# usexfg/xfg-stark

Hardware: AMD Instinct MI355X
Metric: burn-proofs/sec (2^16-step trace, blowup=8) (higher is better)
Workload: dtype u64; 1 GPU; batch of 64 burn proofs per GPU (configs[2]; configs[3] = 512 proofs on 8 GPUs); trace_length=65536, blowup=8, proof_options=42/8/4/None/8/31, parallelism=dp1 (independent proofs; RCCL scatter of inputs, gather of proof bytes), submission=pipelined, depth 6 (xfg_prove_batch_submit / xfg_batch_wait)

## Files before the change

### include/xfg_stark.h

```cpp
#ifndef XFG_STARK_H
#define XFG_STARK_H
#include <stddef.h>
#include <stdint.h>
#ifdef __cplusplus
extern "C" {
#endif

typedef struct xfg_ctx xfg_ctx;

typedef enum {
    XFG_OK = 0,
    XFG_INVALID_BURN_AMOUNT = 1,
    XFG_MINT_MISMATCH = 2,
    XFG_ZERO_TX_HASH = 3,
    XFG_BAD_RECIPIENT_LEN = 4,
    XFG_SHORT_SECRET = 5,
    XFG_PROVER_ERROR = 6,
    XFG_DEVICE_ERROR = 7,
    XFG_BUFFER_TOO_SMALL = 8,
    XFG_INVALID_ARGUMENT = 9,
    XFG_VERIFY_FAILED = 10,
    XFG_INVALID_TRACE = 11
} xfg_status;

// ... 135 lines not shown
                             const uint64_t* coeffs, const uint32_t* coin_seeds, const uint64_t* coin_counters,
                             uint64_t ginv, uint64_t* ood_out, uint64_t* deep_out, uint64_t* dp_out,
                             uint32_t* seeds_out, uint64_t* counters_out, int* fail_out);
int xfg_debug_constraint_eval(xfg_ctx* ctx, uint32_t count, uint64_t n, uint32_t blowup, uint32_t ext,
                              const uint64_t* trace, const xfg_air_consts* airs, const uint64_t* coeffs,
                              uint64_t* ce);
int xfg_debug_fri_fold(xfg_ctx* ctx, uint32_t count, uint32_t ext, uint32_t logn, uint32_t logbeta, int coset_major,
                       const uint64_t* vals, const uint64_t* alpha, uint64_t* out);
int xfg_debug_fri_fold_f(xfg_ctx* ctx, uint32_t count, uint32_t ext, uint32_t logn, uint32_t logbeta, int coset_major,
                         uint32_t fold, const uint64_t* vals, const uint64_t* alpha, uint64_t* out);
int xfg_debug_coin_draws(xfg_ctx* ctx, const uint32_t seed[8], uint64_t counter, uint32_t k, uint32_t ext,
                         const uint64_t reject[4], uint64_t* out_wave, uint64_t* out_seq, uint64_t counters[2],
                         int ok[2]);
int xfg_debug_merkle_lde(xfg_ctx* ctx, uint32_t count, uint32_t nc, uint64_t n, uint32_t blowup, const uint64_t* lde,
                         const uint64_t* entries, uint64_t nentries, uint8_t* nodes_out, uint8_t* local_out);
int xfg_debug_merkle_lde_const(xfg_ctx* ctx, uint32_t count, uint32_t nc, uint64_t n, uint32_t blowup,
                               const uint64_t* lde, const uint8_t* flags, const uint64_t* vals,
                               const uint64_t* entries, uint64_t nentries, uint8_t* nodes_out, uint8_t* local_out);
int xfg_debug_poison_lde(xfg_ctx* ctx, int on);
int xfg_debug_merkle_fri(xfg_ctx* ctx, uint32_t count, uint32_t ext, uint32_t logn, uint32_t logbeta, int coset_major,
                         const uint64_t* vals, uint8_t* nodes_out);
int xfg_debug_merkle_fri_f(xfg_ctx* ctx, uint32_t count, uint32_t ext, uint32_t logn, uint32_t logbeta, int coset_major,
                           uint32_t fold, const uint64_t* vals, uint8_t* nodes_out);
int xfg_debug_grind(xfg_ctx* ctx, uint32_t count, const uint32_t* seeds, uint32_t grind, uint64_t first_nonce,
                    uint64_t max_nonce, uint32_t chunk_log, uint32_t blocks, uint64_t* nonces_out);
int xfg_grind_probe(const xfg_ctx* ctx, uint32_t* device_min, uint64_t* device_searches, uint64_t* host_searches);
int xfg_debug_verify_batch_gpu(xfg_ctx* ctx, uint32_t count, const uint8_t* const* proofs, const size_t* lens,
                               const xfg_air_consts* airs, const xfg_options* acceptable, int* results,
                               uint64_t* flags, char* errs, size_t err_stride);

#ifdef __cplusplus
}
#endif
#endif
```

### xfg-stark_amd/csrc/debug_abi.hip

```cpp
#include <cstring>
#include <vector>

#include "dev_coin.hpp"
#include "dispatch.hpp"
#include "field_dft.hpp"
#include "prover_internal.hpp"

using namespace xfg;

__global__ void field_op_kernel(int op, const u64* a, const u64* b, u64* out, u64 count) {
    const u64 i = (u64)blockIdx.x * blockDim.x + threadIdx.x;
    if (i >= count) return;
    const u64 x = a[i], y = b[i];
    u64 r = 0;
    switch (op) {
        case 0: r = gl_mul(x, y); break;
        case 1: r = gl_add(x, y); break;
        case 2: r = gl_sub(x, y); break;
        case 3: r = gl_canon(x); break;
        case 4: {
            const int sh = (int)(y % 96);
            static_for<96>([&](auto sc) {
                if (sh == decltype(sc)::value) r = mul_pow2<decltype(sc)::value>(x);
            });
// ... 722 lines not shown
        c->err = "xfg_debug_merkle_fri: null or unsupported argument";
        return XFG_INVALID_ARGUMENT;
    }
    return on_lane0(c, [&](Lane* L) -> int {
        const size_t B = count;
        const u64 D = 1ULL << (logn + logbeta), rows = D / fold;
        if (!all_canonical(vals, B * ext * D)) {
            c->err = "layer value is not a canonical field element";
            return XFG_INVALID_ARGUMENT;
        }
        L->f0.ensure(B * ext * D);
        L->tnodes.ensure(B * 2 * rows);
        hipStream_t s = L->stream;
        HIPCHK(hipMemcpyAsync(L->f0.p, vals, B * ext * D * 8, hipMemcpyHostToDevice, s));
        HIPCHK(hipMemsetAsync(L->tnodes.p, 0xFF, B * 2 * rows * sizeof(Digest), s));
        launch_merkle_fri(L->f0.p, ext * D, D, coset_major != 0, (int)logn, (int)logbeta, rows, L->tnodes.p, (int)B,
                          (int)ext, (int)fold, s);
        HIPCHK(hipMemcpyAsync(nodes_out, L->tnodes.p, B * 2 * rows * sizeof(Digest), hipMemcpyDeviceToHost, s));
        HIPCHK(hipStreamSynchronize(s));
        return XFG_OK;
    });
}

}
```

### xfg-stark_amd/csrc/kernels.hip

```cpp
#include "dev_coin.hpp"
#include "dispatch.hpp"
#include "field_dft.hpp"
#include "hip_util.hpp"
#include <algorithm>
#include <stdexcept>

namespace xfg {

__device__ __forceinline__ u64 shfl_xor_u64(u64 v, int m, int w) {
    u32 lo = __shfl_xor((u32)v, m, w), hi = __shfl_xor((u32)(v >> 32), m, w);
    return (u64)lo | ((u64)hi << 32);
}

struct CeArgs {
    const u64* lde;
    const AirConst* air;
    const u64* coeffs;
    const u64* div;
    u64* ce;
    int logn, logbeta;
    ColConst cc;
    const CeUniform* uni;
};
template <int D>
__global__ __launch_bounds__(64) void ce_uniform_kernel(const AirConst* air, const u64* coeffs, ColConst cc,
// ... 497 lines not shown
    while (ct < nblk) ct <<= 1;
    const dim3 g(nblk, npoly), b(T);
    with_ext(ext, [&](auto D) {
        XFG_LAUNCH(deep_carry_kernel<D>, dim3(npoly), dim3(ct), 0, s, partial, dp, carry, nblk, logch);
        with_bool(cc.flags != nullptr, [&](auto CC) {
            XFG_LAUNCH((deep_final_kernel<D, CC>), g, b, 0, s, coef, hcoef, dp, carry, deep, logn, cc);
        });
    });
}

struct FoldArgs {
    const u64* vals;
    u64 val_stride, comp_stride;
    int coset_major, logn, logbeta;
    u64 rows;
    int logD;
    const u64* alpha7;
    u64* out;
    u64 out_stride;
    Tables T;
};
template <int D, int LOGF>
__global__ __launch_bounds__(256) void fri_fold_kernel(FoldArgs a) {
    using F = FE<D>;
    constexpr int NF = 1 << LOGF;
    const int proof = blockIdx.y;
    const u64 i = (u64)blockIdx.x * blockDim.x + threadIdx.x;
    if (i >= a.rows) return;
    const u64* base = a.vals + (u64)proof * a.val_stride;
    u64 c[D][NF];
#pragma unroll
    for (int k = 0; k < NF; k++) {
        const u64 K = i + (u64)k * a.rows;
        c[0][k] = layer_at(base, a.coset_major, a.logn, a.logbeta, K);
        if constexpr (D == 2) c[1][k] = layer_at(base + a.comp_stride, a.coset_major, a.logn, a.logbeta, K);
    }
    F v[NF];
#pragma unroll
    for (int d = 0; d < D; d++) {
        dft_reg<LOGF, true>(c[d]);
#pragma unroll
        for (int k = 0; k < NF; k++) {
            if (d == 0) v[k].a = canon(c[d][k]);
            if constexpr (D == 2) if (d == 1) v[k].b = canon(c[d][k]);
        }
    }
    const F y = fe_mulb(F::load(a.alpha7 + (u64)proof * D), tw_get(a.T, a.logD, i, true));
    F r = v[NF - 1];
#pragma unroll
    for (int j = NF - 2; j >= 0; j--) r = fe_add(fe_mul(r, y), v[j]);
#pragma unroll
    for (int d = 0; d < D; d++) {
        const u64 x = gl_neg(mul_pow2<96 - LOGF>(r.c(d)));
        if (d == 0) r.a = x;
        if constexpr (D == 2) if (d == 1) r.b = x;
    }
#pragma unroll
    for (int c = 0; c < D; c++) a.out[((u64)proof * D + c) * a.out_stride + i] = r.c(c);
}
void launch_fri_fold(const u64* vals, u64 val_stride, u64 comp_stride, bool coset_major, int logn, int logbeta,
                     u64 rows, int logD, const u64* alpha7, u64* out, u64 out_stride, const Tables& T, int npoly,
                     int ext, int fold, hipStream_t s) {
    FoldArgs a;
    a.vals = vals; a.val_stride = val_stride; a.comp_stride = comp_stride; a.coset_major = coset_major ? 1 : 0;
    a.logn = logn; a.logbeta = logbeta; a.rows = rows; a.logD = logD; a.alpha7 = alpha7; a.out = out;
    a.out_stride = out_stride;
    a.T = T;
    int threads = rows < 256 ? (int)rows : 256;
    dim3 g((unsigned)((rows + threads - 1) / threads), npoly);
    with_ext(ext, [&](auto D) {
        with_fold(fold, [&](auto LOGF) { XFG_LAUNCH((fri_fold_kernel<D, LOGF>), g, dim3(threads), 0, s, a); });
    });
}

__global__ void gather_set_kernel(GatherSet g, const u64* idx) {
    const u64 i = (u64)blockIdx.x * blockDim.x + threadIdx.x;
    if (i >= g.first[g.nseg]) return;
    int k = 0;
    while (i >= g.first[k + 1]) k++;
    const u64 src = idx[i];
    if (g.digest[k]) {
// ... 35 lines not shown
```

### xfg-stark_amd/csrc/kernels.hpp

```cpp
#pragma once
#include <hip/hip_runtime.h>
#include "gl.hpp"
#include "air.hpp"
#include "blake3.hpp"
#include "ntt_plan.hpp"
#include "columns.hpp"

namespace xfg {

struct DeepParams {
    u64 a[7][2];
    u64 gamma[2];
    u64 z[2], zg[2], zinv[2], zginv[2];
    u64 c1[2], c2[2];
    u64 pad[2];
};

struct FourStep {
    const u64* fwd[FOURSTEP_MAX_LOG + 1][5] = {};
    const u64* inv[FOURSTEP_MAX_LOG + 1] = {};
    const u64* pass_fwd[PASS_MAX_LOG + 1][5] = {};
};
struct Tables {
    const u64* tw;
    int LM;
    const u64* pow7;
    const u64* ipow7;
    const FourStep* fs;
// ... 45 lines not shown
__host__ __device__ constexpr u64 trace_key(unsigned kind, u64 step, unsigned index) {
    return ((u64)kind << 62) | (step << 3) | index;
}
void launch_trace_check(u64* trace, const AirConst* air, u64* keys, int logn, int npoly, bool with_air, hipStream_t s);
void launch_constraint_eval(const u64* lde, const AirConst* air, const u64* coeffs, const u64* div, u64* ce, int logn,
                            int logbeta, int npoly, int ext, hipStream_t s, const ColConst& cc = ColConst{},
                            CeUniform* uni = nullptr);

void launch_ood(const u64* coef, const u64* hcoef, const u64* zpts, u64* partial, u64* ood, int logn, int npoly,
                int ext, hipStream_t s, const DeepCoinStep& dc = DeepCoinStep{}, const ColConst& cc = ColConst{});
u64 ood_partial_count(int logn);
void launch_deep(const u64* coef, const u64* hcoef, const DeepParams* dp, const u64* partial, u64* carry, u64* deep,
                 int logn, int npoly, int ext, hipStream_t s, const ColConst& cc = ColConst{});

__device__ __forceinline__ u64 layer_at(const u64* base, bool coset_major, int logn, int logbeta, u64 K) {
    if (!coset_major) return base[K];
    u64 t = K & ((1ULL << logbeta) - 1), m = K >> logbeta;
    return base[(t << logn) + m];
}
void launch_fri_fold(const u64* vals, u64 val_stride, u64 comp_stride, bool coset_major, int logn, int logbeta,
                     u64 rows, int logD, const u64* alpha7, u64* out, u64 out_stride, const Tables& T, int npoly,
                     int ext, int fold, hipStream_t s);

struct GatherSet {
    static constexpr int MAX = 24;
    int nseg = 0;
    const void* src[MAX];
    void* dst[MAX];
    int digest[MAX];
    u64 first[MAX + 1] = {0};
    int cc_seg = -1, cc_shift = 0;
    ColConst cc;
};
void launch_gather_set(const GatherSet& g, const u64* idx, hipStream_t s);

struct PackSet {
    static constexpr int MAX = 12;
    int nseg = 0;
    const void* src[MAX];
    u64 off[MAX], words[MAX];
};
void launch_pack(const PackSet& p, void* dst, hipStream_t s);

constexpr size_t grind_state_words(size_t B) { return 2 * ((B + 1) & ~(size_t)1); }
void launch_grind(const Digest* seeds, u64* state, u64* out, unsigned B, unsigned grind, u64 first, u64 max_nonce,
                  unsigned chunk_log, unsigned blocks, hipStream_t s);
// ... 3 lines not shown
```

### xfg-stark_amd/csrc/lane_unit.hip

```cpp
#include <algorithm>
#include <chrono>
#include <cstring>

#include "host_pool.hpp"
#include "prover_internal.hpp"

namespace xfg {

static void stage_mark(Lane* c, int k, hipStream_t on = nullptr) {
    if (c->timing) HIPCHK(hipEventRecord(c->ev[k], on ? on : c->stream));
}

static hipStream_t gather_stream(Lane* c) {
    if (!c->gstream) {
        int least = 0, greatest = 0;
        if (hipDeviceGetStreamPriorityRange(&least, &greatest) != hipSuccess) greatest = 0;
        HIPCHK(hipStreamCreateWithPriority(&c->gstream, hipStreamNonBlocking, greatest));
    }
    return c->gstream;
}

void size_trace_lde(Lane* c, size_t B, const ProofShape& sh) {
    c->trace.ensure(B * 7 * sh.n);
    c->coef.ensure(B * 7 * sh.n);
// ... 130 lines not shown
    if (generated) {
        launch_trace_probe(c->air.p, B, sh.logn, c->const_col.p, c->const_val.p, s);
        launch_trace_gen(c->air.p, B, sh.logn, c->const_col.p, c->trace.p, s);
    } else {
        launch_const_detect(c->trace.p, B * 7, sh.logn, c->const_col.p, s, 7, c->const_val.p);
    }
    launch_interpolate(c->trace.p, sh.n, c->coef.p, sh.n, c->scratch.p, B * 7, sh.logn, false, sh.n, T, s, skip);
    if (probe) {
        if (!c->lde_ev[0]) {
            HIPCHK(hipEventCreate(&c->lde_ev[0]));
            HIPCHK(hipEventCreate(&c->lde_ev[1]));
        }
        HIPCHK(hipEventRecord(c->lde_ev[0], s));
    }
    launch_lde(c->coef.p, sh.n, c->lde.p, c->scratch.p, B * 7, sh.logn, sh.logbeta, T, s, skip);
    if (probe) HIPCHK(hipEventRecord(c->lde_ev[1], s));
}

static void enqueue_fri_layers(Lane* c, const Tables& T, int B, const ProofShape& sh, int fold, CoinStep& cs,
                               HostTrace& ht) {
    hipStream_t s = c->stream;
    const int DE = sh.DE;
    const unsigned nl = sh.nl;
    for (unsigned l = 0; l < nl; l++) {
        const u64 rows = sh.D[l] / fold;
        const bool cm = (l == 0);
        const u64* src = cm ? c->f0.p : c->flayer[l].p;
        const u64 cstride = cm ? sh.N : sh.D[l], sstride = DE * cstride;
        cs.kind = CoinStep::FRI_ALPHA;
        cs.out = c->alpha7.p;
        cs.hist = c->falpha.p + (size_t)l * B * DE;
        cs.root_out = c->droots.p + (size_t)(2 + l) * B;
        launch_merkle_fri(src, sstride, cstride, cm, sh.logn, sh.logbeta, rows, c->fnodes[l].p, B, DE, fold, s, cs);
        launch_fri_fold(src, sstride, cstride, cm, sh.logn, sh.logbeta, rows, (int)ilog2(sh.D[l]), c->alpha7.p,
                        c->flayer[l + 1].p, rows, T, B, DE, fold, s);
    }
    ht.mark("chain_launch");
    if (nl > 0) {
        launch_interpolate(c->flayer[nl].p, sh.D[nl], c->rem.p, sh.rem_len, c->scratch.p, B * DE,
                           (int)ilog2(sh.D[nl]), true, sh.rem_len, T, s);
    } else {
        HIPCHK(hipMemcpy2DAsync(c->rem.p, sh.rem_len * 8, c->deep.p, sh.n * 8, sh.rem_len * 8, (size_t)B * DE,
                                hipMemcpyDeviceToDevice, s));
    }
}

static ReplayView pack_replay_block(Lane* c, size_t B, const ProofShape& sh, bool with_keys) {
    const size_t DE = sh.DE, nl = sh.nl;
    PackSet pk;
    u64 words = 0;
    auto seg = [&](const void* src, size_t bytes) {
        const u64 at = words;
        pk.src[pk.nseg] = src;
        pk.off[pk.nseg] = at;
        pk.words[pk.nseg++] = bytes / 4;
// ... 278 lines not shown
```

### xfg-stark_amd/csrc/merkle.hip

```cpp
#include "dev_coin.hpp"
#include "dispatch.hpp"
#include "hip_util.hpp"
#include <algorithm>
#include <stdexcept>
#include <type_traits>

namespace xfg {

constexpr u64 ROW2_MIN_N = 1024, ROW2_MAX_BLOCKS = 1024;
constexpr int LEAF_LANES_LOG = 1;
constexpr int UP_WMIN = 64;
constexpr int TREE_MID_WMIN = 64, TREE_MID_SHRINK = 8;
constexpr u64 MID4_MAX_BLOCKS = 256;
constexpr u64 TREE_TOP_MAX = 512;

__device__ __forceinline__ void lds_level(Digest& d, bool have, int slot, Digest* lds, int half, Digest* dst) {
    const int t = threadIdx.x;
    if (have) lds[slot] = d;
    __syncthreads();
    if (t < half) {
        d = b3_merge(lds[2 * t], lds[2 * t + 1]);
        dst[t] = d;
    }
}
__device__ __forceinline__ void block_tree_up(Digest d, Digest* nodes, u64 count, Digest* lds, int wmin) {
    u64 c = count;
    for (int w = blockDim.x; w > wmin; w >>= 1) {
        c >>= 1;
        lds_level(d, true, threadIdx.x, lds, w / 2, nodes + c + (u64)blockIdx.x * (w / 2));
        __syncthreads();
    }
}
__device__ __forceinline__ void quad_level(const Digest* src, bool act, int i, int q, Digest* lds, Digest* dst) {
    uint2 o = make_uint2(0, 0);
    if (act) {
        uint32_t m[16];
#pragma unroll
// ... 169 lines not shown
        for (int w = 0; w < 8; w++) r.w[w] = __shfl_xor(d.w[w], 1 << (k - 1 - LPL));
        d = b3_merge(d, r);
        if ((t & ((1 << k) - 1)) == 0) local[((1 << LOGB) + t) >> k] = d;
    }
}

template <class F>
static void with_lde_kernel(int nc, int logbeta, const ColConst& cc, F f) {
    if (cc.flags && nc != 7) throw std::invalid_argument("Merkle kernels: constant columns are those of a 7-column trace LDE");
    if (cc.flags) with_logbeta<7>(logbeta, [&](auto NC, auto LB) { f(NC, LB, std::true_type{}); });
    else with_nc_logbeta(nc, logbeta, [&](auto NC, auto LB) { f(NC, LB, std::false_type{}); });
}

void launch_open_rows(const u64* lde, int nc, const u64* entries, u64 count, Digest* out, int logn, int logbeta,
                      hipStream_t s, const ColConst& cc) {
    if (!count) return;
    const int logl = logbeta < 6 ? logbeta : 6;
    dim3 g((unsigned)(((count << logl) + 63) / 64)), b(64);
    with_lde_kernel(nc, logbeta, cc, [&](auto NC, auto LB, auto CC) {
        XFG_LAUNCH((open_rows_kernel<NC, LB, CC>), g, b, 0, s, lde, entries, count, out, logn, cc);
    });
}

__device__ void coin_root_step(const CoinStep& cs, int b, const Digest& root) {
    const int D = cs.ext, lane = threadIdx.x;
    DevCoin c = cs.coins[b];
    dev_reseed(c, root);
    bool ok;
    if (cs.kind == CoinStep::COEFFS) {
        ok = wave_draw_e(c, 15, D, cs.out + (u64)b * 15 * D, D);
    } else {
        u64 a[2] = {0, 0};
        ok = dev_draw_e(c, a, D);
        if (cs.kind == CoinStep::OOD_POINT) {
            if (a[0] == 0 && a[1] == 0) ok = false;
            if (lane == 0)
                for (int k = 0; k < D; k++) {
                    cs.out[(u64)b * 2 * D + k] = a[k];
                    cs.out[(u64)b * 2 * D + D + k] = gl_mul(a[k], cs.g);
                }
        } else if (lane == 0) {
            const u64 inv7 = 0x249249246DB6DB6EULL;
            for (int k = 0; k < D; k++) cs.out[(u64)b * D + k] = gl_mul(a[k], inv7);
            if (cs.hist)
                for (int k = 0; k < D; k++) cs.hist[(u64)b * D + k] = a[k];
        }
    }
    if (lane == 0) {
        if (!ok) cs.fail[b] = 1;
        cs.coins[b] = c;
        if (cs.root_out) cs.root_out[b] = root;
    }
}

__global__ __launch_bounds__(1024) void tree_top_kernel(Digest* nodes_all, u64 node_stride, u64 count, CoinStep cs) {
    __shared__ Digest lds[256];
    Digest* nodes = nodes_all + (u64)blockIdx.x * node_stride;
    const int tid = threadIdx.x, i = tid >> 2, q = tid & 3;
    for (u64 c = count; c > 1; c >>= 1) {
        const u64 half = c >> 1;
        quad_level(c == count ? nodes + c : lds, i < (int)half, i, q, lds, nodes + half);
    }
    if (cs.kind != CoinStep::NONE && tid < 64) coin_root_step(cs, blockIdx.x, count > 1 ? lds[0] : nodes[1]);
}
__global__ __launch_bounds__(256) void tree_mid_kernel(Digest* nodes_all, u64 node_stride, u64 count) {
    __shared__ Digest lds[256];
    Digest* nodes = nodes_all + (u64)blockIdx.y * node_stride;
    const u64 i = (u64)blockIdx.x * 256 + threadIdx.x;
    const Digest d = b3_merge(nodes[count + 2 * i], nodes[count + 2 * i + 1]);
    nodes[count / 2 + i] = d;
    block_tree_up(d, nodes, count / 2, lds, TREE_MID_WMIN);
}
__global__ __launch_bounds__(256) void tree_mid4_kernel(Digest* nodes_all, u64 node_stride, u64 count) {
    __shared__ Digest lds[64];
    Digest* nodes = nodes_all + (u64)blockIdx.y * node_stride;
    const int tid = threadIdx.x, i = tid >> 2, q = tid & 3;
    u64 c = count, first = (u64)blockIdx.x * 64;
    for (int w = 64; w >= 16; w >>= 1, c >>= 1, first >>= 1)
        quad_level(w == 64 ? nodes + c + 2 * first : lds, i < w, i, q, lds, nodes + c / 2 + first);
}
static void finish_tree(Digest* nodes, u64 node_stride, u64 count, int npoly, hipStream_t s, const CoinStep& cs) {
    while (count > TREE_TOP_MAX) {
        if ((count / 512) * (u64)npoly < MID4_MAX_BLOCKS)
            XFG_LAUNCH(tree_mid4_kernel, dim3((unsigned)(count / 128), npoly), dim3(256), 0, s, nodes, node_stride, count);
        else
            XFG_LAUNCH(tree_mid_kernel, dim3((unsigned)(count / 512), npoly), dim3(256), 0, s, nodes, node_stride, count);
        count /= TREE_MID_SHRINK;
    }
    if (count > 1 || cs.kind != CoinStep::NONE) {
        int threads = (int)(2 * count);
        threads = threads < 64 ? 64 : threads;
        XFG_LAUNCH(tree_top_kernel, dim3(npoly), dim3(threads), 0, s, nodes, node_stride, count, cs);
    }
}

void launch_merkle_lde(const u64* lde, int nc, Digest* nodes, int npoly, int logn, int logbeta, hipStream_t s,
                       const CoinStep& cs, const ColConst& cc) {
    const u64 n = 1ULL << logn, node_stride = 2 * n;
    const bool row2 = n >= ROW2_MIN_N && (u64)npoly * (n / 256) < ROW2_MAX_BLOCKS;
    const int logl = logbeta < LEAF_LANES_LOG ? logbeta : LEAF_LANES_LOG;
    const unsigned T = (unsigned)std::min<u64>(256, n);
    const dim3 g(row2 ? (unsigned)(n >> (8 - logl)) : (unsigned)(n / T), npoly), b(row2 ? 256 : T);
    with_lde_kernel(nc, logbeta, cc, [&](auto NC, auto LB, auto CC) {
        if (row2) XFG_LAUNCH((leaves_row2_kernel<NC, LB, CC>), g, b, 0, s, lde, nodes, node_stride, logn, cc);
        else XFG_LAUNCH((leaves_row_kernel<NC, LB, CC>), g, b, 0, s, lde, nodes, node_stride, logn, cc);
    });
    finish_tree(nodes, node_stride, n / 4, npoly, s, cs);
}

template <int D, int LOGF>
__global__ __launch_bounds__(256) void fri_leaves_kernel(const u64* vals, u64 val_stride, u64 comp_stride,
                                                         int coset_major, int logn, int logbeta, u64 rows,
                                                         Digest* nodes_all, u64 node_stride, int wmin) {
    __shared__ Digest lds[256];
// ... 6 lines not shown
    for (int k = 0; k < NF; k++)
#pragma unroll
        for (int c = 0; c < D; c++)
            v[k * D + c] = layer_at(base + c * comp_stride, coset_major, logn, logbeta, i + (u64)k * rows);
    Digest d = b3_hash_elems<NF * D>(v);
    Digest* nodes = nodes_all + (u64)proof * node_stride;
    nodes[rows + i] = d;
    block_tree_up(d, nodes, rows, lds, wmin);
}
void launch_merkle_fri(const u64* vals, u64 val_stride, u64 comp_stride, bool coset_major, int logn, int logbeta,
                       u64 rows, Digest* nodes, int npoly, int ext, int fold, hipStream_t s, const CoinStep& cs) {
    const u64 T = std::min<u64>(256, rows), node_stride = 2 * rows;
    const int wmin = (int)std::min<u64>(T, UP_WMIN);
    dim3 g((unsigned)(rows / T), npoly);
    with_ext(ext, [&](auto D) {
        with_fold(fold, [&](auto LOGF) {
            XFG_LAUNCH((fri_leaves_kernel<D, LOGF>), g, dim3((unsigned)T), 0, s, vals, val_stride, comp_stride,
                       coset_major ? 1 : 0, logn, logbeta, rows, nodes, node_stride, wmin);
        });
    });
    finish_tree(nodes, node_stride, rows / T * wmin, npoly, s, cs);
}

}
```

### xfg-stark_amd/xfgstark/_abi.py

```python
import ctypes as C
import os

_PKG = os.path.dirname(os.path.dirname(os.path.abspath(__file__)))
LIB_PATH = os.environ.get("XFG_LIB") or os.path.join(_PKG, "libxfgstark.so")
HEADER_PATH = os.path.join(os.path.dirname(_PKG), "include", "xfg_stark.h")

if not os.path.exists(LIB_PATH):
    raise ImportError(f"libxfgstark.so not built at {LIB_PATH}: run `make -C xfg-stark_amd` "
                      "(or __graft_entry__.build()); the prover has no CPU fallback")

_lib = C.CDLL(LIB_PATH)

STATUS = {0: "OK", 1: "INVALID_BURN_AMOUNT", 2: "MINT_MISMATCH", 3: "ZERO_TX_HASH", 4: "BAD_RECIPIENT_LEN",
          5: "SHORT_SECRET", 6: "PROVER_ERROR", 7: "DEVICE_ERROR", 8: "BUFFER_TOO_SMALL", 9: "INVALID_ARGUMENT",
          10: "VERIFY_FAILED", 11: "INVALID_TRACE"}
TRACE_VALIDATE, TRACE_ON_DEVICE = 1, 2


class XfgStarkError(Exception):

    def __init__(self, status, message):
        super().__init__(message)
        self.status = status
        self.kind = STATUS.get(status, str(status))
# ... 71 lines not shown
    ("xfg_bench_lde", _int, [_ctx, _u32, _u64, _u32, _u32, _f64p]),
    ("xfg_lde_probe", _int, [_ctx, _int, _f64p, _u64p, _u64p]),
    ("xfg_debug_lde", _int, [_ctx, _u64p, _u32, _u64, _u32, _u64p]),
    ("xfg_debug_interpolate", _int, [_ctx, _u64p, _u32, _u64, _int, _u64p]),
    ("xfg_debug_const_columns", _int, [_ctx, _u64p, _u32, _u32, _u64, _u8p]),
    ("xfg_debug_col_classes", _int, [_ctx, _u64p, _u32, _u64, _u8p, _u64p]),
    ("xfg_debug_trace_probe", _int, [_ctx, _u32, _u64, _airs, _u32, C.POINTER(_ProbePattern), _u8p, _u64p, _u64p]),
    ("xfg_debug_lde_skip", _int, [_ctx, _u64p, _u32, _u64, _u32, _u8p, _u64p]),
    ("xfg_debug_interpolate_skip", _int, [_ctx, _u64p, _u32, _u64, _int, _u8p, _u64p]),
    ("xfg_debug_interpolate_keep", _int, [_ctx, _u64p, _u32, _u64, _u64, _int, _u64p]),
    ("xfg_debug_field", _int, [_ctx, _u32, _u64, _u64p, _u64p, _u64p]),
    ("xfg_debug_ood_deep", _int, [_ctx, _u32, _u64, _u64p, _u64p, _u64p, _u64p, _u64p, _u64p]),
    ("xfg_debug_ood_deep_e", _int, [_ctx, _u32, _u64, _u32, _u64p] + _OOD_TAIL),
    ("xfg_debug_ood_deep_const", _int, [_ctx, _u32, _u64, _u32, _u64p, _u8p, _u64p] + _OOD_TAIL),
    ("xfg_debug_constraint_eval", _int, [_ctx, _u32, _u64, _u32, _u32, _u64p, _airs, _u64p, _u64p]),
    ("xfg_debug_fri_fold", _int, _FRI + [_u64p, _u64p, _u64p]),
    ("xfg_debug_fri_fold_f", _int, _FRI + [_u32, _u64p, _u64p, _u64p]),
    ("xfg_debug_coin_draws", _int, [_ctx, _u32p, _u64, _u32, _u32, _u64p, _u64p, _u64p, _u64p, _intp]),
    ("xfg_debug_merkle_lde", _int, [_ctx, _u32, _u32, _u64, _u32, _u64p, _u64p, _u64, _u8p, _u8p]),
    ("xfg_debug_merkle_lde_const", _int, [_ctx, _u32, _u32, _u64, _u32, _u64p, _u8p, _u64p, _u64p, _u64, _u8p, _u8p]),
    ("xfg_debug_poison_lde", _int, [_ctx, _int]),
    ("xfg_debug_merkle_fri", _int, _FRI + [_u64p, _u8p]),
    ("xfg_debug_merkle_fri_f", _int, _FRI + [_u32, _u64p, _u8p]),
    ("xfg_debug_grind", _int, [_ctx, _u32, _u32p, _u32, _u64, _u64, _u32, _u32, _u64p]),
    ("xfg_grind_probe", _int, [_ctx, _u32p, _u64p, _u64p]),
    ("xfg_debug_verify_batch_gpu", _int, [_ctx, _u32, _bufs, _szp, _airs, _opts, _intp, _u64p, _str, _sz]),
]


def bind(lib, table=TABLE):
    missing = []
    for name, restype, argtypes in table:
        fn = getattr(lib, name, None)
        if fn is None:
            missing.append(name)
        else:
            fn.restype, fn.argtypes = restype, argtypes
    return missing


MISSING = bind(_lib)


def exported_symbols():
    return dir(_lib)
```

### xfg-stark_amd/xfgstark/_hooks.py

```python
import ctypes as C

from ._abi import XfgStarkError, _lib, _ProbePattern, _u8p, _u32p
from ._marshal import air_array, array, ptr, words, zeros


class KernelHooks:

    def debug_lde(self, coef, n, blowup):
        c = array(coef).reshape(-1, n)
        out = zeros((c.shape[0], n * blowup))
        self._call(_lib.xfg_debug_lde, ptr(c), c.shape[0], n, blowup, ptr(out))
        return out

    def debug_lde_skip(self, coef, n, blowup, skip):
        c = array(coef).reshape(-1, n)
        f = array(skip, "uint8", (c.shape[0],), "debug_lde_skip: one flag per polynomial")
        out = zeros((c.shape[0], n * blowup))
        self._call(_lib.xfg_debug_lde_skip, ptr(c), c.shape[0], n, blowup, ptr(f, _u8p), ptr(out))
        return out

    def debug_const_columns(self, trace):
        tr = array(trace)
        B, width, n = tr.shape
        out = zeros((B, width), "uint8")
# ... 131 lines not shown
            if f.shape != (B, nc) or cv.shape != (B, nc):
                raise XfgStarkError(9, "debug_merkle_lde_const: flags [B,nc], vals [B,nc]")
            fp, vp = ptr(f, _u8p), ptr(cv)
        nodes, local = zeros((B, 2 * n, 8), "<u4"), zeros((ent.size, 2 * blowup, 8), "<u4")
        self._call(_lib.xfg_debug_merkle_lde_const, B, nc, n, blowup, ptr(v), fp, vp, ptr(ent), ent.size,
                   ptr(nodes, _u8p), ptr(local, _u8p))
        return nodes, local

    def debug_poison_lde(self, on):
        self._call(_lib.xfg_debug_poison_lde, 1 if on else 0)

    def debug_merkle_fri(self, vals, logn, logbeta, coset_major, fold=8):
        v = array(vals)
        B, ext, D = v.shape
        if D != 1 << (logn + logbeta):
            raise XfgStarkError(9, "debug_merkle_fri: vals [B,ext,2^(logn+logbeta)]")
        if not 0 < fold < 1 << 32:
            raise XfgStarkError(9, "debug_merkle_fri: fold is 2, 4, 8 or 16")
        nodes = zeros((B, 2 * (D // fold), 8), "<u4")
        self._call(_lib.xfg_debug_merkle_fri_f, B, ext, logn, logbeta, 1 if coset_major else 0, fold, ptr(v),
                   ptr(nodes, _u8p))
        return nodes

    def debug_interpolate(self, evals, n, offset7=False):
        e = array(evals).reshape(-1, n)
        out = zeros(e.shape)
        self._call(_lib.xfg_debug_interpolate, ptr(e), e.shape[0], n, 1 if offset7 else 0, ptr(out))
        return out

    def debug_interpolate_keep(self, evals, n, keep, offset7=False):
        e = array(evals).reshape(-1, n)
        keep = int(keep)
        if not 0 <= keep < 1 << 64:
            raise XfgStarkError(9, "debug_interpolate_keep: keep is 1..n")
        out = zeros(e.shape[0] * min(keep, n) + 8)
        self._call(_lib.xfg_debug_interpolate_keep, ptr(e), e.shape[0], n, keep, 1 if offset7 else 0, ptr(out))
        return out[:-8].reshape(e.shape[0], keep), out[-8:]

    def debug_interpolate_skip(self, evals, n, skip, offset7=False):
        e = array(evals).reshape(-1, n)
        f = array(skip, "uint8", (e.shape[0],), "debug_interpolate_skip: one flag per polynomial")
        out = zeros(e.shape)
        self._call(_lib.xfg_debug_interpolate_skip, ptr(e), e.shape[0], n, 1 if offset7 else 0, ptr(f, _u8p), ptr(out))
        return out
```

Before: 22710 proofs/s.

## Fuse small FRI tail layers into one per-proof kernel with commit, alpha draw and fold

After: 22640 proofs/s. About the same (-0.3%).

```diff
diff --git a/include/xfg_stark.h b/include/xfg_stark.h
--- a/include/xfg_stark.h
+++ b/include/xfg_stark.h
@@ -181,6 +181,10 @@
                          const uint64_t* vals, uint8_t* nodes_out);
 int xfg_debug_merkle_fri_f(xfg_ctx* ctx, uint32_t count, uint32_t ext, uint32_t logn, uint32_t logbeta, int coset_major,
                            uint32_t fold, const uint64_t* vals, uint8_t* nodes_out);
+int xfg_debug_fri_tail(xfg_ctx* ctx, uint32_t count, uint32_t ext, uint32_t logn, uint32_t logbeta, int coset_major,
+                       uint32_t fold, uint32_t nlayers, const uint64_t* vals, const uint32_t* seeds,
+                       const uint64_t* counters, uint8_t* nodes_out, uint64_t* alphas_out, uint64_t* layers_out,
+                       uint8_t* roots_out, uint32_t* seeds_out, uint64_t* counters_out, int* fail_out);
 int xfg_debug_grind(xfg_ctx* ctx, uint32_t count, const uint32_t* seeds, uint32_t grind, uint64_t first_nonce,
                     uint64_t max_nonce, uint32_t chunk_log, uint32_t blocks, uint64_t* nonces_out);
 int xfg_grind_probe(const xfg_ctx* ctx, uint32_t* device_min, uint64_t* device_searches, uint64_t* host_searches);
diff --git a/xfg-stark_amd/csrc/debug_abi.hip b/xfg-stark_amd/csrc/debug_abi.hip
--- a/xfg-stark_amd/csrc/debug_abi.hip
+++ b/xfg-stark_amd/csrc/debug_abi.hip
@@ -768,4 +768,97 @@
     });
 }
 
-}
+int xfg_debug_fri_tail(xfg_ctx* c, uint32_t count, uint32_t ext, uint32_t logn, uint32_t logbeta, int coset_major,
+                       uint32_t fold, uint32_t nlayers, const uint64_t* vals, const uint32_t* seeds,
+                       const uint64_t* counters, uint8_t* nodes_out, uint64_t* alphas_out, uint64_t* layers_out,
+                       uint8_t* roots_out, uint32_t* seeds_out, uint64_t* counters_out, int* fail_out) {
+    if (!c) return XFG_INVALID_ARGUMENT;
+    c->err.clear();
+    const unsigned logf = fold_log2(fold);
+    if (!vals || !seeds || !counters || !nodes_out || !alphas_out || !layers_out || !roots_out || !seeds_out ||
+        !counters_out || !fail_out || count == 0 || count > 0xFFFF || (ext != 1 && ext != 2) || logn > 28 ||
+        logbeta > 28 || !logf || logn + logbeta > 28 || nlayers == 0 || nlayers > FRI_TAIL_MAX_LAYERS ||
+        logn + logbeta < nlayers * logf || (1ULL << (logn + logbeta)) / fold > FRI_TAIL_MAX_ROWS) {
+        c->err = "xfg_debug_fri_tail: null or unsupported argument (first layer of at most 1024 rows, every layer "
+                 "of at least one)";
+        return XFG_INVALID_ARGUMENT;
+    }
+    return on_lane0(c, [&](Lane* L) -> int {
+        const size_t B = count, nl = nlayers;
+        const int logD = (int)(logn + logbeta);
+        const u64 D0 = 1ULL << logD;
+        if (!all_canonical(vals, B * ext * D0)) {
+            c->err = "layer value is not a canonical field element";
+            return XFG_INVALID_ARGUMENT;
+        }
+        std::vector<u64> Ds(nl + 1);
+        for (size_t l = 0; l <= nl; l++) Ds[l] = D0 >> (l * logf);
+        const FriTailPlan tail = fri_tail_plan(Ds.data(), (unsigned)nl, fold);
+        if (tail.first != 0 || tail.layers != nl) {
+            c->err = "xfg_debug_fri_tail: the layers are not one tail";
+            return XFG_INVALID_ARGUMENT;
+        }
+        ensure_tables(c, logD);
+        const Tables T = tables_of(c);
+        L->f0.ensure(B * ext * D0);
+        L->alpha7.ensure(B * ext);
+        L->falpha.ensure(nl * B * ext);
+        L->droots.ensure(nl * B);
+        L->dcoin.ensure(B);
+        L->dfail.ensure(B);
+        if (L->flayer.size() < nl + 1) {
+            L->flayer.resize(nl + 1);
+            L->fnodes.resize(nl + 1);
+        }
+        hipStream_t s = L->stream;
+        Digest* nodes[FRI_TAIL_MAX_LAYERS];
+        u64* out[FRI_TAIL_MAX_LAYERS];
+        for (size_t l = 0; l < nl; l++) {
+            const u64 rows = Ds[l + 1];
+            L->fnodes[l].ensure(B * 2 * rows);
+            L->flayer[l + 1].ensure(B * ext * rows);
+            HIPCHK(hipMemsetAsync(L->fnodes[l].p, 0xFF, B * 2 * rows * sizeof(Digest), s));
+            HIPCHK(hipMemsetAsync(L->flayer[l + 1].p, 0xFF, B * ext * rows * 8, s));
+            nodes[l] = L->fnodes[l].p;
+            out[l] = L->flayer[l + 1].p;
+        }
+        std::vector<DevCoin> hc(B);
+        for (size_t b = 0; b < B; b++) {
+            memcpy(hc[b].seed.w, seeds + 8 * b, 32);
+            hc[b].counter = counters[b];
+            hc[b].pad = 0;
+        }
+        HIPCHK(hipMemcpyAsync(L->f0.p, vals, B * ext * D0 * 8, hipMemcpyHostToDevice, s));
+        HIPCHK(hipMemcpyAsync(L->dcoin.p, hc.data(), B * sizeof(DevCoin), hipMemcpyHostToDevice, s));
+        HIPCHK(hipMemsetAsync(L->dfail.p, 0, B * sizeof(int), s));
+        HIPCHK(hipMemsetAsync(L->alpha7.p, 0xFF, B * ext * 8, s));
+        HIPCHK(hipMemsetAsync(L->falpha.p, 0xFF, nl * B * ext * 8, s));
+        HIPCHK(hipMemsetAsync(L->droots.p, 0xFF, nl * B * sizeof(Digest), s));
+        CoinStep cs;
+        cs.ext = (int)ext;
+        cs.coins = L->dcoin.p;
+        cs.fail = L->dfail.p;
+        cs.out = L->alpha7.p;
+        launch_fri_tail(L->f0.p, ext * D0, D0, coset_major != 0, (int)logn, (int)logbeta, tail.rows, (int)nl, tail.block,
+                        nodes, out, L->falpha.p, L->droots.p, cs, T, (int)B, (int)ext, (int)fold, s);
+        for (size_t l = 0; l < nl; l++) {
+            const u64 rows = Ds[l + 1];
+            HIPCHK(hipMemcpyAsync(nodes_out, nodes[l], B * 2 * rows * sizeof(Digest), hipMemcpyDeviceToHost, s));
+            HIPCHK(hipMemcpyAsync(layers_out, out[l], B * ext * rows * 8, hipMemcpyDeviceToHost, s));
+            nodes_out += B * 2 * rows * sizeof(Digest);
+            layers_out += B * ext * rows;
+        }
+        HIPCHK(hipMemcpyAsync(alphas_out, L->falpha.p, nl * B * ext * 8, hipMemcpyDeviceToHost, s));
+        HIPCHK(hipMemcpyAsync(roots_out, L->droots.p, nl * B * sizeof(Digest), hipMemcpyDeviceToHost, s));
+        HIPCHK(hipMemcpyAsync(hc.data(), L->dcoin.p, B * sizeof(DevCoin), hipMemcpyDeviceToHost, s));
+        HIPCHK(hipMemcpyAsync(fail_out, L->dfail.p, B * sizeof(int), hipMemcpyDeviceToHost, s));
+        HIPCHK(hipStreamSynchronize(s));
+        for (size_t b = 0; b < B; b++) {
+            memcpy(seeds_out + 8 * b, hc[b].seed.w, 32);
+            counters_out[b] = hc[b].counter;
+        }
+        return XFG_OK;
+    });
+}
+
+}
diff --git a/xfg-stark_amd/csrc/fri_fold.hpp b/xfg-stark_amd/csrc/fri_fold.hpp
--- /dev/null
+++ b/xfg-stark_amd/csrc/fri_fold.hpp
@@ -0,0 +1,44 @@
+#pragma once
+#include "field_dft.hpp"
+#include "kernels.hpp"
+
+namespace xfg {
+
+template <int D, int LOGF>
+__device__ __forceinline__ void fri_fold_row(const u64* base, u64 comp_stride, bool coset_major, int logn, int logbeta,
+                                             u64 rows, int logD, FE<D> alpha7, const Tables& T, u64 i, u64* out,
+                                             u64 out_stride) {
+    using F = FE<D>;
+    constexpr int NF = 1 << LOGF;
+    u64 c[D][NF];
+#pragma unroll
+    for (int k = 0; k < NF; k++) {
+        const u64 K = i + (u64)k * rows;
+        c[0][k] = layer_at(base, coset_major, logn, logbeta, K);
+        if constexpr (D == 2) c[1][k] = layer_at(base + comp_stride, coset_major, logn, logbeta, K);
+    }
+    F v[NF];
+#pragma unroll
+    for (int d = 0; d < D; d++) {
+        dft_reg<LOGF, true>(c[d]);
+#pragma unroll
+        for (int k = 0; k < NF; k++) {
+            if (d == 0) v[k].a = canon(c[d][k]);
+            if constexpr (D == 2) if (d == 1) v[k].b = canon(c[d][k]);
+        }
+    }
+    const F y = fe_mulb(alpha7, tw_get(T, logD, i, true));
+    F r = v[NF - 1];
+#pragma unroll
+    for (int j = NF - 2; j >= 0; j--) r = fe_add(fe_mul(r, y), v[j]);
+#pragma unroll
+    for (int d = 0; d < D; d++) {
+        const u64 x = gl_neg(mul_pow2<96 - LOGF>(r.c(d)));
+        if (d == 0) r.a = x;
+        if constexpr (D == 2) if (d == 1) r.b = x;
+    }
+#pragma unroll
+    for (int c2 = 0; c2 < D; c2++) out[(u64)c2 * out_stride + i] = r.c(c2);
+}
+
+}
diff --git a/xfg-stark_amd/csrc/fri_tail_plan.hpp b/xfg-stark_amd/csrc/fri_tail_plan.hpp
--- /dev/null
+++ b/xfg-stark_amd/csrc/fri_tail_plan.hpp
@@ -0,0 +1,29 @@
+#pragma once
+#include <stdint.h>
+
+namespace xfg {
+
+constexpr uint64_t FRI_TAIL_MAX_ROWS = 1024;
+constexpr unsigned FRI_TAIL_BLOCK_MAX = 256, FRI_TAIL_BLOCK_MIN = 64;
+constexpr unsigned FRI_TAIL_MAX_LAYERS = 12;
+
+struct FriTailPlan {
+    unsigned first;
+    unsigned layers;
+    unsigned block;
+    uint64_t rows;
+};
+
+constexpr FriTailPlan fri_tail_plan(const uint64_t* D, unsigned nl, uint64_t fold, uint64_t max_rows = FRI_TAIL_MAX_ROWS) {
+    unsigned first = 0;
+    while (first < nl && D[first] / fold > max_rows) first++;
+    if (nl - first > FRI_TAIL_MAX_LAYERS) first = nl - FRI_TAIL_MAX_LAYERS;
+    if (first == nl) return FriTailPlan{nl, 0, 0, 0};
+    const uint64_t rows = D[first] / fold;
+    const unsigned block = rows >= FRI_TAIL_BLOCK_MAX ? FRI_TAIL_BLOCK_MAX
+                           : rows <= FRI_TAIL_BLOCK_MIN ? FRI_TAIL_BLOCK_MIN
+                                                        : (unsigned)rows;
+    return FriTailPlan{first, nl - first, block, rows};
+}
+
+}
diff --git a/xfg-stark_amd/csrc/kernels.hip b/xfg-stark_amd/csrc/kernels.hip
--- a/xfg-stark_amd/csrc/kernels.hip
+++ b/xfg-stark_amd/csrc/kernels.hip
@@ -1,6 +1,7 @@
 #include "dev_coin.hpp"
 #include "dispatch.hpp"
 #include "field_dft.hpp"
+#include "fri_fold.hpp"
 #include "hip_util.hpp"
 #include <algorithm>
 #include <stdexcept>
@@ -544,41 +545,12 @@
 };
 template <int D, int LOGF>
 __global__ __launch_bounds__(256) void fri_fold_kernel(FoldArgs a) {
-    using F = FE<D>;
-    constexpr int NF = 1 << LOGF;
     const int proof = blockIdx.y;
     const u64 i = (u64)blockIdx.x * blockDim.x + threadIdx.x;
     if (i >= a.rows) return;
-    const u64* base = a.vals + (u64)proof * a.val_stride;
-    u64 c[D][NF];
-#pragma unroll
-    for (int k = 0; k < NF; k++) {
-        const u64 K = i + (u64)k * a.rows;
-        c[0][k] = layer_at(base, a.coset_major, a.logn, a.logbeta, K);
-        if constexpr (D == 2) c[1][k] = layer_at(base + a.comp_stride, a.coset_major, a.logn, a.logbeta, K);
-    }
-    F v[NF];
-#pragma unroll
-    for (int d = 0; d < D; d++) {
-        dft_reg<LOGF, true>(c[d]);
-#pragma unroll
-        for (int k = 0; k < NF; k++) {
-            if (d == 0) v[k].a = canon(c[d][k]);
-            if constexpr (D == 2) if (d == 1) v[k].b = canon(c[d][k]);
-        }
-    }
-    const F y = fe_mulb(F::load(a.alpha7 + (u64)proof * D), tw_get(a.T, a.logD, i, true));
-    F r = v[NF - 1];
-#pragma unroll
-    for (int j = NF - 2; j >= 0; j--) r = fe_add(fe_mul(r, y), v[j]);
-#pragma unroll
-    for (int d = 0; d < D; d++) {
-        const u64 x = gl_neg(mul_pow2<96 - LOGF>(r.c(d)));
-        if (d == 0) r.a = x;
-        if constexpr (D == 2) if (d == 1) r.b = x;
-    }
-#pragma unroll
-    for (int c = 0; c < D; c++) a.out[((u64)proof * D + c) * a.out_stride + i] = r.c(c);
+    fri_fold_row<D, LOGF>(a.vals + (u64)proof * a.val_stride, a.comp_stride, a.coset_major, a.logn, a.logbeta, a.rows,
+                          a.logD, FE<D>::load(a.alpha7 + (u64)proof * D), a.T, i, a.out + (u64)proof * D * a.out_stride,
+                          a.out_stride);
 }
 void launch_fri_fold(const u64* vals, u64 val_stride, u64 comp_stride, bool coset_major, int logn, int logbeta,
                      u64 rows, int logD, const u64* alpha7, u64* out, u64 out_stride, const Tables& T, int npoly,
diff --git a/xfg-stark_amd/csrc/kernels.hpp b/xfg-stark_amd/csrc/kernels.hpp
--- a/xfg-stark_amd/csrc/kernels.hpp
+++ b/xfg-stark_amd/csrc/kernels.hpp
@@ -4,6 +4,7 @@
 #include "air.hpp"
 #include "blake3.hpp"
 #include "ntt_plan.hpp"
+#include "fri_tail_plan.hpp"
 #include "columns.hpp"
 
 namespace xfg {
@@ -95,6 +96,10 @@
                      u64 rows, int logD, const u64* alpha7, u64* out, u64 out_stride, const Tables& T, int npoly,
                      int ext, int fold, hipStream_t s);
 
+void launch_fri_tail(const u64* vals, u64 val_stride, u64 comp_stride, bool coset_major, int logn, int logbeta, u64 rows,
+                     int nlayers, unsigned block, Digest* const* nodes, u64* const* out, u64* hist, Digest* roots,
+                     const CoinStep& cs, const Tables& T, int npoly, int ext, int fold, hipStream_t s);
+
 struct GatherSet {
     static constexpr int MAX = 24;
     int nseg = 0;
diff --git a/xfg-stark_amd/csrc/lane_unit.hip b/xfg-stark_amd/csrc/lane_unit.hip
--- a/xfg-stark_amd/csrc/lane_unit.hip
+++ b/xfg-stark_amd/csrc/lane_unit.hip
@@ -176,15 +176,27 @@
     hipStream_t s = c->stream;
     const int DE = sh.DE;
     const unsigned nl = sh.nl;
+    const FriTailPlan tail = fri_tail_plan(sh.D.data(), nl, (u64)fold);
+    cs.kind = CoinStep::FRI_ALPHA;
+    cs.out = c->alpha7.p;
     for (unsigned l = 0; l < nl; l++) {
         const u64 rows = sh.D[l] / fold;
         const bool cm = (l == 0);
         const u64* src = cm ? c->f0.p : c->flayer[l].p;
         const u64 cstride = cm ? sh.N : sh.D[l], sstride = DE * cstride;
-        cs.kind = CoinStep::FRI_ALPHA;
-        cs.out = c->alpha7.p;
         cs.hist = c->falpha.p + (size_t)l * B * DE;
         cs.root_out = c->droots.p + (size_t)(2 + l) * B;
+        if (l == tail.first) {
+            Digest* nodes[FRI_TAIL_MAX_LAYERS];
+            u64* out[FRI_TAIL_MAX_LAYERS];
+            for (unsigned k = 0; k < tail.layers; k++) {
+                nodes[k] = c->fnodes[l + k].p;
+                out[k] = c->flayer[l + k + 1].p;
+            }
+            launch_fri_tail(src, sstride, cstride, cm, sh.logn, sh.logbeta, rows, (int)tail.layers, tail.block, nodes, out,
+                            cs.hist, cs.root_out, cs, T, B, DE, fold, s);
+            break;
+        }
         launch_merkle_fri(src, sstride, cstride, cm, sh.logn, sh.logbeta, rows, c->fnodes[l].p, B, DE, fold, s, cs);
         launch_fri_fold(src, sstride, cstride, cm, sh.logn, sh.logbeta, rows, (int)ilog2(sh.D[l]), c->alpha7.p,
                         c->flayer[l + 1].p, rows, T, B, DE, fold, s);
diff --git a/xfg-stark_amd/csrc/merkle.hip b/xfg-stark_amd/csrc/merkle.hip
--- a/xfg-stark_amd/csrc/merkle.hip
+++ b/xfg-stark_amd/csrc/merkle.hip
@@ -1,5 +1,7 @@
 #include "dev_coin.hpp"
 #include "dispatch.hpp"
+#include "fri_fold.hpp"
+#include "fri_tail_plan.hpp"
 #include "hip_util.hpp"
 #include <algorithm>
 #include <stdexcept>
@@ -13,6 +15,8 @@
 constexpr int TREE_MID_WMIN = 64, TREE_MID_SHRINK = 8;
 constexpr u64 MID4_MAX_BLOCKS = 256;
 constexpr u64 TREE_TOP_MAX = 512;
+constexpr int TOP_BLOCK_MAX = 256;
+constexpr int TOP_WIDE_MAX_TREES = 4;
 
 __device__ __forceinline__ void lds_level(Digest& d, bool have, int slot, Digest* lds, int half, Digest* dst) {
     const int t = threadIdx.x;
@@ -228,7 +232,7 @@
     });
 }
 
-__device__ void coin_root_step(const CoinStep& cs, int b, const Digest& root) {
+__device__ void coin_root_step(const CoinStep& cs, int b, const Digest& root, u64* share = nullptr) {
     const int D = cs.ext, lane = threadIdx.x;
     DevCoin c = cs.coins[b];
     dev_reseed(c, root);
@@ -247,7 +251,11 @@
                 }
         } else if (lane == 0) {
             const u64 inv7 = 0x249249246DB6DB6EULL;
-            for (int k = 0; k < D; k++) cs.out[(u64)b * D + k] = gl_mul(a[k], inv7);
+            for (int k = 0; k < D; k++) {
+                const u64 a7 = gl_mul(a[k], inv7);
+                cs.out[(u64)b * D + k] = a7;
+                if (share) share[k] = a7;
+            }
             if (cs.hist)
                 for (int k = 0; k < D; k++) cs.hist[(u64)b * D + k] = a[k];
         }
@@ -260,14 +268,31 @@
 }
 
 __global__ __launch_bounds__(1024) void tree_top_kernel(Digest* nodes_all, u64 node_stride, u64 count, CoinStep cs) {
-    __shared__ Digest lds[256];
+    __shared__ Digest lds[2][256];
     Digest* nodes = nodes_all + (u64)blockIdx.x * node_stride;
-    const int tid = threadIdx.x, i = tid >> 2, q = tid & 3;
-    for (u64 c = count; c > 1; c >>= 1) {
-        const u64 half = c >> 1;
-        quad_level(c == count ? nodes + c : lds, i < (int)half, i, q, lds, nodes + half);
-    }
-    if (cs.kind != CoinStep::NONE && tid < 64) coin_root_step(cs, blockIdx.x, count > 1 ? lds[0] : nodes[1]);
+    const int tid = threadIdx.x, q = tid & 3, quads = blockDim.x >> 2;
+    int cur = 0;
+    for (u64 c = count; c > 1; c >>= 1, cur ^= 1) {
+        const int half = (int)(c >> 1);
+        const Digest* src = c == count ? nodes + c : lds[cur];
+        Digest *keep = lds[cur ^ 1], *dst = nodes + half;
+#pragma unroll 1
+        for (int i = tid >> 2; i < half; i += quads) {
+            uint32_t m[16];
+#pragma unroll
+            for (int w = 0; w < 8; w++) {
+                m[w] = src[2 * i].w[w];
+                m[8 + w] = src[2 * i + 1].w[w];
+            }
+            const uint2 o = b3_merge_quad(m, q);
+            keep[i].w[q] = o.x;
+            keep[i].w[4 + q] = o.y;
+            dst[i].w[q] = o.x;
+            dst[i].w[4 + q] = o.y;
+        }
+        __syncthreads();
+    }
+    if (cs.kind != CoinStep::NONE && tid < 64) coin_root_step(cs, blockIdx.x, count > 1 ? lds[cur][0] : nodes[1]);
 }
 __global__ __launch_bounds__(256) void tree_mid_kernel(Digest* nodes_all, u64 node_stride, u64 count) {
     __shared__ Digest lds[256];
@@ -296,6 +321,7 @@
     if (count > 1 || cs.kind != CoinStep::NONE) {
         int threads = (int)(2 * count);
         threads = threads < 64 ? 64 : threads;
+        if (npoly >= TOP_WIDE_MAX_TREES && threads > TOP_BLOCK_MAX) threads = TOP_BLOCK_MAX;
         XFG_LAUNCH(tree_top_kernel, dim3(npoly), dim3(threads), 0, s, nodes, node_stride, count, cs);
     }
 }
@@ -348,4 +374,116 @@
     finish_tree(nodes, node_stride, rows / T * wmin, npoly, s, cs);
 }
 
-}
+struct FriTailArgs {
+    const u64* vals;
+    u64 val_stride, comp_stride;
+    int coset_major, logn, logbeta;
+    u64 rows;
+    int logD;
+    int nlayers;
+    Digest* nodes[FRI_TAIL_MAX_LAYERS];
+    u64* out[FRI_TAIL_MAX_LAYERS];
+    u64* hist;
+    Digest* roots;
+    CoinStep cs;
+    Tables T;
+};
+template <int D, int LOGF>
+__device__ __forceinline__ Digest fri_leaf(const u64* base, u64 comp_stride, bool cm, int logn, int logbeta, u64 rows, u64 i) {
+    constexpr int NF = 1 << LOGF;
+    u64 v[NF * D];
+#pragma unroll
+    for (int k = 0; k < NF; k++)
+#pragma unroll
+        for (int c = 0; c < D; c++) v[k * D + c] = layer_at(base + c * comp_stride, cm, logn, logbeta, i + (u64)k * rows);
+    return b3_hash_elems<NF * D>(v);
+}
+template <int D, int LOGF>
+__global__ __launch_bounds__(256) void fri_tail_kernel(FriTailArgs a) {
+    static_assert(FRI_TAIL_MAX_ROWS <= 4 * FRI_TAIL_BLOCK_MAX && FRI_TAIL_BLOCK_MAX <= 256, "at most four rows per lane");
+    __shared__ Digest lds[256];
+    __shared__ u64 alpha_s[2];
+    const int t = threadIdx.x, W = blockDim.x, proof = blockIdx.x, B = gridDim.x;
+    const u64* base = a.vals + (u64)proof * a.val_stride;
+    u64 comp_stride = a.comp_stride, rows = a.rows;
+    bool cm = a.coset_major != 0;
+    int logD = a.logD;
+#pragma unroll 1
+    for (int l = 0; l < a.nlayers; l++) {
+        Digest* nodes = a.nodes[l] + (u64)proof * 2 * rows;
+        const int G = rows > (u64)W ? (int)(rows / W) : 1;
+        const int count = (int)(rows / G);
+        Digest d, p1, p2;
+        if (t < count) {
+#pragma unroll 1
+            for (int j = 0; j < G; j++) {
+                const u64 i = (u64)t * G + j;
+                d = fri_leaf<D, LOGF>(base, comp_stride, cm, a.logn, a.logbeta, rows, i);
+                nodes[rows + i] = d;
+                if (j & 1) {
+                    d = b3_merge(p1, d);
+                    nodes[(rows + i) >> 1] = d;
+                    if (j & 2) {
+                        d = b3_merge(p2, d);
+                        nodes[(rows + i) >> 2] = d;
+                    } else {
+                        p2 = d;
+                    }
+                } else {
+                    p1 = d;
+                }
+            }
+        }
+        int c = count;
+        for (; 4 * (c >> 1) > W; c >>= 1) {
+            lds_level(d, t < c, t, lds, c >> 1, nodes + (c >> 1));
+            __syncthreads();
+        }
+        if (t < c) lds[t] = d;
+        __syncthreads();
+        for (; c > 1; c >>= 1) quad_level(lds, (t >> 2) < (c >> 1), t >> 2, t & 3, lds, nodes + (c >> 1));
+        if (t < 64) {
+            CoinStep cs = a.cs;
+            cs.kind = CoinStep::FRI_ALPHA;
+            cs.hist = a.hist + (u64)l * B * D;
+            cs.root_out = a.roots + (u64)l * B;
+            coin_root_step(cs, proof, lds[0], alpha_s);
+        }
+        __syncthreads();
+        const FE<D> alpha7 = FE<D>::load(alpha_s);
+        u64* out = a.out[l] + (u64)proof * D * rows;
+        for (u64 i = t; i < rows; i += W)
+            fri_fold_row<D, LOGF>(base, comp_stride, cm, a.logn, a.logbeta, rows, logD, alpha7, a.T, i, out, rows);
+        __threadfence_block();
+        __syncthreads();
+        base = out;
+        comp_stride = rows;
+        cm = false;
+        logD -= LOGF;
+        rows >>= LOGF;
+    }
+}
+void launch_fri_tail(const u64* vals, u64 val_stride, u64 comp_stride, bool coset_major, int logn, int logbeta, u64 rows,
+                     int nlayers, unsigned block, Digest* const* nodes, u64* const* out, u64* hist, Digest* roots,
+                     const CoinStep& cs, const Tables& T, int npoly, int ext, int fold, hipStream_t s) {
+    const int logf = fold_log2(fold);
+    if (nlayers < 1 || nlayers > (int)FRI_TAIL_MAX_LAYERS || block < FRI_TAIL_BLOCK_MIN || block > FRI_TAIL_BLOCK_MAX ||
+        (block & (block - 1)) || rows < 1 || (rows & (rows - 1)) || rows > 4 * (u64)block || (rows < block && block != FRI_TAIL_BLOCK_MIN) ||
+        !logf || (rows >> ((nlayers - 1) * logf)) < 1)
+        throw std::invalid_argument("FRI tail: layers or rows outside what one block per proof takes");
+    FriTailArgs a;
+    a.vals = vals; a.val_stride = val_stride; a.comp_stride = comp_stride; a.coset_major = coset_major ? 1 : 0;
+    a.logn = logn; a.logbeta = logbeta; a.rows = rows; a.nlayers = nlayers;
+    a.logD = logf;
+    while ((1ULL << a.logD) < rows * (u64)fold) a.logD++;
+    for (int l = 0; l < (int)FRI_TAIL_MAX_LAYERS; l++) {
+        a.nodes[l] = l < nlayers ? nodes[l] : nullptr;
+        a.out[l] = l < nlayers ? out[l] : nullptr;
+    }
+    a.hist = hist; a.roots = roots; a.cs = cs; a.T = T;
+    with_ext(ext, [&](auto D) {
+        with_fold(fold, [&](auto LOGF) { XFG_LAUNCH((fri_tail_kernel<D, LOGF>), dim3(npoly), dim3(block), 0, s, a); });
+    });
+}
+
+}
diff --git a/xfg-stark_amd/xfgstark/_abi.py b/xfg-stark_amd/xfgstark/_abi.py
--- a/xfg-stark_amd/xfgstark/_abi.py
+++ b/xfg-stark_amd/xfgstark/_abi.py
@@ -117,6 +117,7 @@
     ("xfg_debug_poison_lde", _int, [_ctx, _int]),
     ("xfg_debug_merkle_fri", _int, _FRI + [_u64p, _u8p]),
     ("xfg_debug_merkle_fri_f", _int, _FRI + [_u32, _u64p, _u8p]),
+    ("xfg_debug_fri_tail", _int, _FRI + [_u32, _u32, _u64p, _u32p, _u64p, _u8p, _u64p, _u64p, _u8p, _u32p, _u64p, _intp]),
     ("xfg_debug_grind", _int, [_ctx, _u32, _u32p, _u32, _u64, _u64, _u32, _u32, _u64p]),
     ("xfg_grind_probe", _int, [_ctx, _u32p, _u64p, _u64p]),
     ("xfg_debug_verify_batch_gpu", _int, [_ctx, _u32, _bufs, _szp, _airs, _opts, _intp, _u64p, _str, _sz]),
diff --git a/xfg-stark_amd/xfgstark/_hooks.py b/xfg-stark_amd/xfgstark/_hooks.py
--- a/xfg-stark_amd/xfgstark/_hooks.py
+++ b/xfg-stark_amd/xfgstark/_hooks.py
@@ -177,6 +177,32 @@
                    ptr(nodes, _u8p))
         return nodes
 
+    def debug_fri_tail(self, vals, logn, logbeta, coset_major, fold, nlayers, coins):
+        v = array(vals)
+        B, ext, D = v.shape
+        if D != 1 << (logn + logbeta):
+            raise XfgStarkError(9, "debug_fri_tail: vals [B,ext,2^(logn+logbeta)]")
+        if not (0 < fold < 1 << 32 and 0 < nlayers <= 64 and fold ** nlayers <= D):
+            raise XfgStarkError(9, "debug_fri_tail: fold is 2, 4, 8 or 16 and every layer has a row")
+        if len(coins) != B or any(len(bytes(sd)) != 32 for sd, _ in coins):
+            raise XfgStarkError(9, "debug_fri_tail: coins are B x (32-byte seed, counter)")
+        rows = [D // fold ** (l + 1) for l in range(nlayers)]
+        seeds, ctrs = words(b"".join(bytes(sd) for sd, _ in coins)), array([ctr for _, ctr in coins])
+        nodes, layers = zeros((B * 2 * sum(rows), 8), "<u4"), zeros(B * ext * sum(rows))
+        alphas, roots = zeros((nlayers, B, ext)), zeros((nlayers, B, 8), "<u4")
+        seeds_out, ctrs_out = zeros(B * 8, "<u4"), zeros(B)
+        fail = (C.c_int * B)()
+        self._call(_lib.xfg_debug_fri_tail, B, ext, logn, logbeta, 1 if coset_major else 0, fold, nlayers, ptr(v),
+                   ptr(seeds, _u32p), ptr(ctrs), ptr(nodes, _u8p), ptr(alphas), ptr(layers), ptr(roots, _u8p),
+                   ptr(seeds_out, _u32p), ptr(ctrs_out), fail)
+        node_l, layer_l, no, lo = [], [], 0, 0
+        for r in rows:
+            node_l.append(nodes[no:no + B * 2 * r].reshape(B, 2 * r, 8))
+            layer_l.append(layers[lo:lo + B * ext * r].reshape(B, ext, r))
+            no, lo = no + B * 2 * r, lo + B * ext * r
+        after = [(seeds_out[8 * b:8 * b + 8].tobytes(), int(ctrs_out[b])) for b in range(B)]
+        return node_l, alphas, layer_l, roots, after, [fail[b] for b in range(B)]
+
     def debug_interpolate(self, evals, n, offset7=False):
         e = array(evals).reshape(-1, n)
         out = zeros(e.shape)
```
